# ameya-deshmukh/pbft

Measured on AMD Instinct MI355X. Metric: Ed25519 verifies/sec per node (1M-signature PBFT rounds), higher is better.
Workload: dtype u32 (GF(2^255-19) radix 2^25.5 limbs, 32x32->64 products)

## Files before the change

pbft_amd/csrc/finish.hip:

```cpp
#include <hip/hip_runtime.h>
#include <stdint.h>

#ifndef PBFT_FIN_STAMPS
#define PBFT_FIN_STAMPS 0
#endif
#if PBFT_FIN_STAMPS
#define FIN_STAMP_WAVES 4096
__device__ uint64_t g_fin_stamp[FIN_STAMP_WAVES][12];
#define FIN_STAMP(k) \
  if (lane == 0 && wave < FIN_STAMP_WAVES) g_fin_stamp[wave][k] = __builtin_amdgcn_s_memtime()
extern "C" int pbft_debug_fin_stamps(uint64_t* out, uint32_t waves) {
  if (waves > FIN_STAMP_WAVES) waves = FIN_STAMP_WAVES;
  return (int)hipMemcpyFromSymbol(out, HIP_SYMBOL(g_fin_stamp), sizeof(uint64_t) * 12 * waves, 0,
                                  hipMemcpyDeviceToHost);
}
#else
#define FIN_STAMP(k)
#endif
#include "verify_kernels.h"


template <int FM, int LV, int W>
__global__ void __launch_bounds__(BLOCK, W) finish_kernel(const uint8_t* __restrict__ R,
                                                       uint32_t rs_stride,
                                                       const uint32_t* __restrict__ xyz,
                                                       const uint8_t* __restrict__ flags, uint64_t N,
                                                       uint64_t* __restrict__ bitmap) {
  const int lane = threadIdx.x & 63;
  const uint64_t wave = ((uint64_t)blockIdx.x * BLOCK + threadIdx.x) >> 6;
  constexpr bool PRE = PBFT_FIN_PREFETCH && ((FM <= 4 && W == 1) || FM == 1);
#if FIN_USE_TAB
  __shared__ uint64_t ds_tab[LV > 0 ? DS_TAB_ENTRIES : 1];
  if constexpr (LV > 0) {
    const uint4* src = (const uint4*)g_ds_tab.e;
    uint4* dst = (uint4*)ds_tab;
#pragma unroll
    for (int k = 0; k < DS_TAB_ENTRIES / 2 / BLOCK; ++k) dst[k * BLOCK + threadIdx.x] = src[k * BLOCK + threadIdx.x];
    if (wave * FM * 64 >= N) { __syncthreads(); return; }
  }
#else
  const uint64_t* ds_tab = nullptr;
#endif
  if (wave * FM * 64 >= N) return;
  finish_wave<FM, LV, PRE, true>(wave, lane, R, rs_stride, xyz, flags, N, bitmap, ds_tab);
}


hipError_t launch_finish(int fm, int lv, int w, const uint8_t* R, uint32_t rs_stride, const uint32_t* xyz,
                         const uint8_t* flags, uint64_t N, uint64_t* bitmap, hipStream_t st) {
#define PBFT_LAUNCH_FIN(M_, LV_, W_)                                                                           \
  hipLaunchKernelGGL((finish_kernel<M_, LV_, W_>),                                                          \
                     dim3((unsigned)((((N + 64 * M_ - 1) / (64 * M_)) * 64 + BLOCK - 1) / BLOCK)), dim3(BLOCK), 0, \
                     st, R, rs_stride, xyz, flags, N, bitmap)
  if (lv == 0) {
    if (fm == 16) PBFT_LAUNCH_FIN(16, 0, FIN_WAVES_PER_EU);
    else if (fm == 8) PBFT_LAUNCH_FIN(8, 0, FIN_WAVES_PER_EU);
    else if (fm == 4) PBFT_LAUNCH_FIN(4, 0, FIN_WAVES_PER_EU);
    else if (fm == 2) PBFT_LAUNCH_FIN(2, 0, FIN_WAVES_PER_EU);
    else PBFT_LAUNCH_FIN(1, 0, FIN_WAVES_PER_EU);
  } else if (w >= 2) {
    if (fm >= 8) PBFT_LAUNCH_FIN(8, PBFT_FIN_LV, 2);
    else if (fm == 4) PBFT_LAUNCH_FIN(4, PBFT_FIN_LV, 2);
    else if (fm == 2) PBFT_LAUNCH_FIN(2, PBFT_FIN_LV, 2);
    else PBFT_LAUNCH_FIN(1, PBFT_FIN_LV, 2);
  } else {
    if (fm == 16) PBFT_LAUNCH_FIN(16, PBFT_FIN_LV, 1);
    else if (fm == 8) PBFT_LAUNCH_FIN(8, PBFT_FIN_LV, 1);
    else if (fm == 4) PBFT_LAUNCH_FIN(4, PBFT_FIN_LV, 1);
    else if (fm == 2) PBFT_LAUNCH_FIN(2, PBFT_FIN_LV, 1);
    else PBFT_LAUNCH_FIN(1, PBFT_FIN_LV, 1);
  }
#undef PBFT_LAUNCH_FIN
  return hipGetLastError();
}


// ... 42 lines not shown
```

pbft_amd/csrc/finish_core.h:

```cpp
#pragma once
#include "verify_core.h"

#ifndef FIN_STAMP
#define FIN_STAMP(k)
#endif

__device__ __forceinline__ void load_fe(fe& f, const uint32_t* __restrict__ base, uint64_t N, uint64_t i) {
#pragma unroll
  for (int t = 0; t < 10; ++t) f.v[t] = base[(size_t)t * N + i];
}

template <int M>
struct fin_unroll {
  template <class F>
  __device__ static __forceinline__ void up(F&& f) {
    fin_unroll<M - 1>::up(f);
    f(std::integral_constant<int, M - 1>());
  }
  template <class F>
  __device__ static __forceinline__ void down(F&& f) {
    f(std::integral_constant<int, M - 1>());
    fin_unroll<M - 1>::down(f);
  }
};
// ... 18 lines not shown
#endif
#ifndef PBFT_FIN_PAR
#define PBFT_FIN_PAR 0
#endif
#ifndef PBFT_FIN_DPP
#define PBFT_FIN_DPP 0
#endif
template <int K>
__device__ __forceinline__ uint32_t tree_partner(uint32_t v) {
#if PBFT_FIN_DPP
  if constexpr (K == 0) return (uint32_t)__builtin_amdgcn_mov_dpp((int)v, 0xB1, 0xF, 0xF, false);
  else if constexpr (K == 1) return (uint32_t)__builtin_amdgcn_mov_dpp((int)v, 0x4E, 0xF, 0xF, false);
  else if constexpr (K == 2) return (uint32_t)__builtin_amdgcn_mov_dpp((int)v, 0x141, 0xF, 0xF, false);
  else if constexpr (K == 3) return (uint32_t)__builtin_amdgcn_mov_dpp((int)v, 0x140, 0xF, 0xF, false);
  else if constexpr (K == 4) return (uint32_t)__builtin_amdgcn_ds_swizzle((int)v, (0x10 << 10) | 0x1F);
  else
#endif
    return (uint32_t)__shfl_xor((int)v, 1 << K);
}


template <int FM, int LV, bool PRE, bool SYNC>
__device__ __forceinline__ void finish_wave(uint64_t wave, int lane, const uint8_t* __restrict__ R, uint32_t rs_stride,
                                            const uint32_t* __restrict__ xyz, const uint8_t* __restrict__ flags,
                                            uint64_t N, uint64_t* __restrict__ bitmap, const uint64_t* ds_tab) {
  (void)ds_tab; (void)flags;
  const uint64_t base = wave * FM * 64 + lane;
  FIN_STAMP(0);
#if PBFT_FIN_STAMPS && defined(FIN_STAMP_WAVES)
  if (lane == 0 && wave < FIN_STAMP_WAVES) g_fin_stamp[wave][6] = __builtin_amdgcn_s_memrealtime();
#endif
  const uint32_t* Xb = xyz;
  const uint32_t* Yb = xyz + 10 * N;
  const uint32_t* Zb = xyz + 20 * N;
  fe pre[FM];
  fe zs[PRE ? FM : 1], xs[PRE ? FM : 1], ys[PRE ? FM : 1];
  constexpr bool PRE_R = PRE && PBFT_FIN_PREFETCH_R;
  uint32_t rs[PRE_R ? FM : 1][8];
  bool fls[PRE_R ? FM : 1];
  fin_unroll<FM>::up([&](auto mc) {
    constexpr int m = decltype(mc)::value;
    const uint64_t i = base + (uint64_t)m * 64;
    fe z;
    if (i < N) load_fe(z, Zb, N, i); else fe_one(z);
    if constexpr (PRE) {
      zs[m] = z;
      const uint64_t ii = i < N ? i : 0;
      load_fe(xs[m], Xb, N, ii);
      load_fe(ys[m], Yb, N, ii);
      if constexpr (PRE_R) {
        load32(rs[m], R + (size_t)rs_stride * ii);
        fls[m] = flags[ii];
      }
    }
    if constexpr (m == 0) pre[0] = z;
    else fe_mulT<PBFT_FIN_PAR>(pre[m], pre[m - 1], z);
  });
  FIN_STAMP(1);
  fe inv;
  fe tq[LV > 0 ? LV : 1];
  fe t = pre[FM - 1];
  static_for<LV>([&](auto kc) {
    constexpr int k = decltype(kc)::value;
#pragma unroll
    for (int u = 0; u < 10; ++u) tq[k].v[u] = tree_partner<k>(t.v[u]);
    fe_mulT<PBFT_FIN_PAR>(t, t, tq[k]);
  });
  FIN_STAMP(2);
#if PBFT_ABL_NOINV
  inv = t;
#elif PBFT_FIN_EXP
  fe_invert<true>(inv, t);
#else
  if constexpr (LV > 0) {
#if FIN_USE_TAB
// ... 10 lines not shown
    fe_invert_var(inv, t, prof);
    if (lane == 0 && wave < FIN_STAMP_WAVES) {
      g_fin_stamp[wave][8] = prof[0]; g_fin_stamp[wave][9] = prof[1]; g_fin_stamp[wave][10] = prof[2];
    }
#else
    static_assert(LV == 6, "");
    fe_invert_var(inv, t);
#endif
  } else {
    fe_invert_gcd(inv, t);
  }
#endif
  FIN_STAMP(3);
  static_for<LV>([&](auto kc) {
    constexpr int k = LV - 1 - decltype(kc)::value;
    fe_mulT<PBFT_FIN_PAR>(inv, inv, tq[k]);
  });
  FIN_STAMP(4);
  fin_unroll<FM>::down([&](auto mc) {
    constexpr int m = decltype(mc)::value;
    const uint64_t i = base + (uint64_t)m * 64;
    const bool live = i < N;
    const uint64_t ii = live ? i : 0;
    fe zi;
    if constexpr (m > 0) {
      fe_mulT<PBFT_FIN_PAR>(zi, inv, pre[m - 1]);
      fe z;
      if constexpr (PRE) z = zs[m];
      else if (live) load_fe(z, Zb, N, ii); else fe_one(z);
      fe_mulT<PBFT_FIN_PAR>(inv, inv, z);
    } else {
      zi = inv;
    }
    fe X, Y, x, y;
    if constexpr (PRE) {
      X = xs[m];
      Y = ys[m];
    } else {
      load_fe(X, Xb, N, ii);
      load_fe(Y, Yb, N, ii);
    }
    bool fl;
    uint32_t r[8];
    if constexpr (PRE_R) {
      fl = fls[m];
#pragma unroll
      for (int t = 0; t < 8; ++t) r[t] = rs[m][t];
    } else {
      fl = flags[ii];
      load32(r, R + (size_t)rs_stride * ii);
    }
    fe_mulT<PBFT_FIN_PAR>(x, X, zi);
    fe_mulT<PBFT_FIN_PAR>(y, Y, zi);
    uint32_t xw[8], yw[8], ry[8];
    fe_to_words(xw, x);
    fe_to_words(yw, y);
    canon_y(ry, r);
    bool eq = (xw[0] & 1u) == (r[7] >> 31);
#pragma unroll
    for (int t = 0; t < 8; ++t) eq = eq && yw[t] == ry[t];
    const bool ok = live && fl && eq && !y_is_small_order(yw);
    const uint64_t vote = __ballot(ok);
    if (lane == 0 && live) bitmap[(wave * FM + m)] = vote;
  });
  FIN_STAMP(5);
#if PBFT_FIN_STAMPS && defined(FIN_STAMP_WAVES)
  if (lane == 0 && wave < FIN_STAMP_WAVES) g_fin_stamp[wave][7] = __builtin_amdgcn_s_memrealtime();
#endif
}
```

pbft_amd/csrc/pbft_verify.hip:

```cpp
#include <dlfcn.h>
#include <sched.h>
#include <hip/hip_runtime.h>
#include <sys/mman.h>
#include <rccl/rccl.h>
#include <stdio.h>
#include <stdlib.h>
#include <string.h>

#include <algorithm>
#include <atomic>
#include <chrono>
#include <mutex>
#include <random>
#include <string>
#include <type_traits>
#include <vector>

#include "../../include/pbft_verify.h"
#include "../../include/pbft_wire.h"
#include "../../include/pbft_replica.h"
#include "digest_kernels.h"
#include "verify_core.h"

using namespace pbft;
// ... 340 lines not shown
    if (c->d_stage) HIP_TRY(hipFree(c->d_stage));
    c->d_stage = nullptr;
    size_t cap = bytes + (bytes >> 2) + 4096;
    if (hipMalloc(&c->d_stage, cap) != hipSuccess) { c->stage_cap = 0; return set_err(PBFT_ENOMEM, "staging alloc"); }
    c->stage_cap = cap;
  }
  if (words > c->bitmap_cap) {
    if (c->d_bitmap) HIP_TRY(hipFree(c->d_bitmap));
    if (c->h_bitmap) HIP_TRY(hipHostFree(c->h_bitmap));
    c->d_bitmap = nullptr; c->h_bitmap = nullptr; c->h_bitmap_dev = nullptr;
    size_t cap = words + 64;
    if (hipMalloc(&c->d_bitmap, cap * 8) != hipSuccess) return set_err(PBFT_ENOMEM, "bitmap alloc");
    if (hipHostMalloc(&c->h_bitmap, cap * 8, hipHostMallocMapped | hipHostMallocCoherent) != hipSuccess)
      return set_err(PBFT_ENOMEM, "pinned bitmap alloc");
    HIP_TRY(hipHostGetDevicePointer((void**)&c->h_bitmap_dev, c->h_bitmap, 0));
    c->bitmap_cap = cap;
  }
  return PBFT_OK;
}

static constexpr int MAX_STEPS = steps<PLB, PLA_SMALL>::N;
static_assert(steps<PLB, PLA_SMALL>::N >= steps<PLB, PLA_MID>::N && steps<PLB, PLA_MID>::N >= steps<PLB, PLA_BIG>::N,
              "");
static inline size_t eidx_offset(uint64_t N) { return (121 * (size_t)N + 255) & ~(size_t)255; }
static inline size_t eidx_bytes(uint64_t N) {
  const uint64_t Npad = (N + 2 * BLOCK - 1) / (2 * BLOCK) * (2 * BLOCK);
  const size_t split4 = 8 * (size_t)((MAX_STEPS + 3) / 4) * (Npad * 4 + BLOCK);
  const size_t split8 = 8 * (size_t)((MAX_STEPS + 7) / 8) * (Npad * 8 + BLOCK);
  const size_t split = split4 > split8 ? split4 : split8;
  const size_t comb = 4 * (size_t)MAX_STEPS * Npad;
  return ((comb > split ? comb : split) + 255) & ~(size_t)255;
}
static double launch_trace_ms() {
  static const double ms = [] {
    const char* e = getenv("PBFT_LAUNCH_TRACE");
    if (!e) return -1.0;
    const double v = strtod(e, nullptr);
    return v > 1 ? v / 1000.0 : 0.3;
  }();
  return ms;
}
static bool launch_trace() { return launch_trace_ms() >= 0; }
#define LT(name, ...)                                                                                              \
  do {                                                                                                             \
    const auto lt_t0 = std::chrono::steady_clock::now();                                                           \
    __VA_ARGS__;                                                                                                   \
    if (launch_trace()) {                                                                                          \
// ... 51 lines not shown
                         const uint32_t* dMI = nullptr, uint32_t n_msg = 0, const uint64_t* dWK = nullptr,
                         uint32_t mi_stride = 1, int slot = 0) {
  if (N == 0) return PBFT_OK;
  const uint64_t blocks = (N + BLOCK - 1) / BLOCK;
  if (blocks > 0x7fffffffull) return set_err(PBFT_EINVAL, "N too large for one launch");
  int rc = slot ? ensure_work2(c, N) : ensure_work(c, N, fst != nullptr);
  if (rc) return rc;
  uint8_t* const wbase = slot ? c->d_work2 : c->d_work;
  const bool timing = c->timing && slot == 0;
  int h = 0;
  if (fst) {
    h = c->half;
    c->half ^= 1;
  }
  if (slot == 0 && c->fin_pending[h]) HIP_TRY(hipStreamWaitEvent(st, c->ev_fin[h], 0));
  if (timing) LT("rec_ev0", HIP_TRY(hipEventRecord(c->ev0, st)));
  const uint64_t W = slot ? c->work2_n : c->work_n;
  uint8_t* hw = wbase + (h ? half1_offset(W) : 0);
  const bool latency_mode = N < c->split_below;
  comb_launch_args a;
  a.R = dR; a.S = dS; a.K = (const uint8_t*)dK; a.rs_stride = rs_stride; a.k_stride = k_stride;
  a.M = dM; a.msg_len = msg_len; a.msg_stride = msg_stride; a.N = N;
  a.tabB = c->d_tabB; a.tabA = c->d_tabA; a.keys = c->d_keys; a.key_ok = c->d_key_ok; a.n_keys = c->n_keys;
  a.xyz = (uint32_t*)hw;
  a.flags = hw + 120 * N;
  a.eidx = (uint32_t*)(wbase + eidx_offset(W));
  a.bitmap = dB; a.msg_idx = dMI; a.n_msg = n_msg; a.mi_stride = mi_stride; a.latency_mode = latency_mode; a.lat_split = c->lat_split; a.st = st;
  a.pair = c->comb_pair;
  a.cus = c->cus;
  a.prio = c->comb_prio;
  a.balance = c->comb_balance;
  a.wk = (PBFT_ENV_SCHED && dMI && msg_len == PBFT_ENVELOPE_LEN) ? dWK : nullptr;
  uint32_t* xyz = a.xyz;
  uint8_t* flags = a.flags;
  LT("comb", HIP_TRY(c->pa == PLA_HUGE::P  ? launch_comb_huge(a)
                     : c->pa == PLA_BIG::P ? launch_comb_big(a)
                     : c->pa == PLA_MID::P ? launch_comb_mid(a)
                                           : launch_comb_small(a)));
  HIP_TRY(hipGetLastError());
  if (fst) {
    if (timing) HIP_TRY(hipEventRecord(c->ev1, st));
    HIP_TRY(hipEventRecord(c->ev_comb, st));
    HIP_TRY(hipStreamWaitEvent(fst, c->ev_comb, 0));
    st = fst;
  }
  if (!latency_mode) {
    const bool big = N >= ((uint64_t)1 << 19);
    int fm = big ? PBFT_FIN_FM_BIG : N > PBFT_FIN_SMALL_UPTO ? PBFT_FIN_FM_MID
                                   : N > PBFT_FIN_TINY_UPTO  ? PBFT_FIN_FM_SMALL : 1;
    int lv = fm <= PBFT_FIN_TREE_MAX_FM ? PBFT_FIN_LV : 0;
    if (c->fin_m) fm = c->fin_m;
    if (c->fin_tree >= 0) lv = c->fin_tree;
    const int fw = c->fin_waves ? c->fin_waves : (big ? PBFT_FIN_W_BIG : 1);
    LT("finish", HIP_TRY(launch_finish(fm, lv, fw, dR, rs_stride, xyz, flags, N, dB, st)));
    HIP_TRY(hipGetLastError());
  }
  if (fst) {
    HIP_TRY(hipEventRecord(c->ev_fin[h], fst));
    c->fin_pending[h] = true;
    return PBFT_OK;
  }
  if (timing) LT("rec_ev1", HIP_TRY(hipEventRecord(c->ev1, st)));
  return PBFT_OK;
}

static bool check_batch_args(const void* R, const void* S, const void* K, const void* M, uint32_t msg_len,
                             uint32_t msg_stride, uint64_t N, const void* out) {
  if (N == 0) return out != nullptr || true;
  if (!R || !S || !K || !out) return false;
  if (msg_len > 0 && !M) return false;
  if (msg_stride < msg_len) return false;
  if (msg_len > (1u << 24)) return false;
  return true;
}

struct stage_layout {
  size_t offS, offK, offM, bytes;
// ... 2339 lines not shown
```

pbft_amd/csrc/verify_core.h:

```cpp
#pragma once
#include "ge25519.h"
#include "inv25519.h"
#include "sc25519.h"
#include "sha512.h"

#include <type_traits>

namespace pbft {

template <int P_, int W_, int NB_ = 0>
struct plan {
  static_assert(P_ * W_ + NB_ >= 254 && NB_ <= P_, "windows must cover 254 bits");
  static constexpr int P = P_;
  __host__ __device__ static constexpr int width(int pos) { return pos < NB_ ? W_ + 1 : W_; }
  __host__ __device__ static constexpr uint32_t entries(int pos) { return (1u << (width(pos) - 1)) + 1u; }
  __host__ __device__ static constexpr uint32_t offset(int pos) {
    return pos <= NB_ ? (uint32_t)pos * ((1u << W_) + 1u)
                      : (uint32_t)NB_ * ((1u << W_) + 1u) + (uint32_t)(pos - NB_) * ((1u << (W_ - 1)) + 1u);
  }
  __host__ __device__ static constexpr int bitoff(int pos) {
    return pos <= NB_ ? pos * (W_ + 1) : NB_ * (W_ + 1) + (pos - NB_) * W_;
  }
  static constexpr uint32_t ENTRIES = offset(P_);
  static constexpr int ENTRY_WORDS = 32;
// ... 42 lines not shown
  }
}

FE_FN uint32_t lane_mask(bool c) {
  uint32_t m = 0u - (uint32_t)c;
#if defined(__HIP_DEVICE_COMPILE__)
  asm("" : "+v"(m));
#endif
  return m;
}

#ifndef PBFT_MADD_V2
#define PBFT_MADD_V2 1
#endif
#ifndef PBFT_CHAIN_MIN_N
#define PBFT_CHAIN_MIN_N (1u << 16)
#endif
FE_FN void fe_cneg_canon(fe& out, const fe& k, uint32_t m) {
  fe nk;
  fe_neg(nk, k);
#pragma unroll
  for (int i = 0; i < 10; ++i) out.v[i] = (k.v[i] & ~m) | (nk.v[i] & m);
}
template <bool WITH_T = true, bool CHAIN = false>
FE_FN void ge_madd_ab(ge& r, const ge& p, const fe& qa, const fe& qb, const fe& k, bool neg) {
#if PBFT_MADD_V2
  fe a, b, c, t, kk;
  fe_cneg_canon(kk, k, lane_mask(neg));
  fe_sub(t, p.Y, p.X);
  if constexpr (CHAIN) {
    fe t2;
    fe_add(t2, p.Y, p.X);
    {
      fe* const ho[3] = {&a, &b, &c};
      const fe* const fo[3] = {&t, &t2, &p.T};
      const fe* const go[3] = {&qa, &qb, &kk};
      fe_mul_chain<3>(ho, fo, go);
    }
  } else {
    fe_mul(a, t, qa);
    fe_add(t, p.Y, p.X);
    fe_mul(b, t, qb);
    fe_mul(c, p.T, kk);
  }
  fe e, f, g, h;
  fe_sub(e, b, a);
  fe_sub(f, p.Z, c);
  fe_add(g, p.Z, c);
  fe_add(h, b, a);
  if constexpr (CHAIN && WITH_T) {
    fe* const ho[4] = {&r.X, &r.Y, &r.Z, &r.T};
    const fe* const fo[4] = {&f, &h, &f, &h};
    const fe* const go[4] = {&e, &g, &g, &e};
    fe_mul_chain<4>(ho, fo, go);
  } else if constexpr (CHAIN) {
    fe* const ho[3] = {&r.X, &r.Y, &r.Z};
    const fe* const fo[3] = {&f, &h, &f};
    const fe* const go[3] = {&e, &g, &g};
    fe_mul_chain<3>(ho, fo, go);
  } else {
    fe_mul(r.X, f, e);
    fe_mul(r.Y, h, g);
    fe_mul(r.Z, f, g);
    if constexpr (WITH_T) fe_mul(r.T, h, e);
  }
#else
  fe a, b, c, t;
  const uint32_t m = lane_mask(neg);
  fe_sub(t, p.Y, p.X);
  fe_mul(a, t, qa);
  fe_add(t, p.Y, p.X);
  fe_mul(b, t, qb);
// ... 89 lines not shown
#pragma unroll
  for (int i = 0; i < 8; ++i) {
    z = z && y[i] == 0u;
    one = one && y[i] == (i == 0 ? 1u : 0u);
    m1 = m1 && y[i] == (i == 0 ? 0xffffffecu : (i == 7 ? 0x7fffffffu : 0xffffffffu));
    a8 = a8 && y[i] == Y8A[i];
    b8 = b8 && y[i] == Y8B[i];
  }
  return z || one || m1 || a8 || b8;
}

FE_FN void canon_y(uint32_t y[8], const uint32_t enc[8]) {
#pragma unroll
  for (int i = 0; i < 8; ++i) y[i] = enc[i];
  y[7] &= 0x7fffffffu;
  bool ge = y[7] == 0x7fffffffu && y[0] >= 0xffffffedu;
#pragma unroll
  for (int i = 1; i < 7; ++i) ge = ge && y[i] == 0xffffffffu;
  if (ge) {
    y[0] -= 0xffffffedu;
#pragma unroll
    for (int i = 1; i < 8; ++i) y[i] = 0;
  }
}

template <int N, int I = 0, class F>
FE_FN void static_for(F&& f) {
  if constexpr (I < N) {
    f(std::integral_constant<int, I>());
    static_for<N, I + 1>(f);
  }
}

template <class PLB, class PLA, int LEN>
FE_FN bool verify_lane(const uint32_t r_enc[8], const uint32_t s[8], const uint32_t a_enc[8], bool key_ok,
                       const uint8_t* msg, int len, const uint32_t* tabB, const uint32_t* tabA) {
  const bool s_ok = sc_lt_L(s);
  uint32_t h[16], k[8];
  sha512_ram<LEN>(h, r_enc, a_enc, msg, len);
  sc_reduce512(k, h);

  ge P;
  digits ds, dk;
  uint32_t sc[8];
#pragma unroll
  for (int i = 0; i < 8; ++i) sc[i] = s[i];
// ... 112 lines not shown
```

pbft_amd/csrc/verify_kernels.h:

```cpp
#pragma once
#include <hip/hip_runtime.h>
#include <stdint.h>

#include <type_traits>

#include "verify_core.h"

using namespace pbft;


#define PBFT_ENVELOPE_LEN 85
#define BLOCK 256
#ifndef PBFT_PLAN_B
#define PBFT_PLAN_B 10, 25, 4
#endif
#ifndef PBFT_PLAN_A
#define PBFT_PLAN_A 14, 18, 2
#endif
using PLB = plan<PBFT_PLAN_B>;
using PLA_HUGE = plan<13, 19, 7>;
using PLA_BIG = plan<PBFT_PLAN_A>;
using PLA_MID = plan<16, 15, 14>;
using PLA_SMALL = plan<32, 7, 30>;
static_assert(PLA_HUGE::P < PLA_BIG::P && PLA_BIG::P < PLA_MID::P && PLA_MID::P < PLA_SMALL::P,
// ... 154 lines not shown
  }
}

#ifndef PBFT_COMB_STAMPS
#define PBFT_COMB_STAMPS 0
#endif
#if PBFT_COMB_STAMPS
#define COMB_STAMP_WAVES 16384
static __device__ uint64_t g_comb_stamp[COMB_STAMP_WAVES][8];
#define COMB_T() __builtin_amdgcn_s_memtime()
#define COMB_RT() __builtin_amdgcn_s_memrealtime()
#endif

static constexpr uint32_t COMB_PRIO_LDS = 64;
#ifndef PBFT_COMB_BALANCE
#define PBFT_COMB_BALANCE -1
#endif
template <int LEN, class PLA, bool CHAIN = false, int WPB = 4, bool BAL = false>
__global__ void __launch_bounds__(64 * WPB, PBFT_COMB_WAVES_PER_EU) comb_kernel(
    const uint8_t* __restrict__ R, const uint8_t* __restrict__ S, const uint8_t* __restrict__ key_idx,
    uint32_t rs_stride, uint32_t k_stride,
    const uint8_t* __restrict__ msg, uint32_t msg_len, uint32_t msg_stride, uint64_t N, uint64_t Npad,
    const uint32_t* __restrict__ tabB, const uint32_t* __restrict__ tabA, const uint32_t* __restrict__ keys,
    const uint8_t* __restrict__ key_ok, uint32_t n_keys, uint32_t* __restrict__ xyz, uint8_t* __restrict__ flags,
    uint32_t* __restrict__ eidx, const uint32_t* __restrict__ msg_idx, uint32_t n_msg, uint32_t mi_stride,
    const uint64_t* __restrict__ wk) {
  using ST = steps<PLB, PLA>;
  extern __shared__ __attribute__((aligned(16))) uint8_t lds[];
  const int lane = threadIdx.x & 63;
  const uint32_t wave = __builtin_amdgcn_readfirstlane(threadIdx.x >> 6);
  const uint32_t ebuf = (uint32_t)(uintptr_t)lds + wave * COMB_LDS_PER_WAVE;
  const uint64_t i = (uint64_t)blockIdx.x * (64 * WPB) + threadIdx.x;
  const bool live = i < N;
  const uint64_t ii = live ? i : 0;
  typename ST::mask_t sgn = 0;
  bool s_ok, kok;
  constexpr bool PRIO = WPB == 8;
  static_assert(!(PRIO && BAL), "the paired-priority form sets its priorities from its partner's progress");
  constexpr int BAL_J1 = ST::N / 3, BAL_J2 = 2 * ST::N / 3;
  if constexpr (BAL) __builtin_amdgcn_s_setprio(3);
  const uint32_t prog = (uint32_t)(uintptr_t)lds + WPB * COMB_LDS_PER_WAVE;
  if constexpr (PRIO) {
    if (lane == 0) lds_write32(prog + 4u * wave, 0u);
    __syncthreads();
  }
#if PBFT_COMB_STAMPS
  const uint64_t st_t0 = COMB_T(), st_rt0 = COMB_RT();
// ... 101 lines not shown
    }
    COMB_WAIT_VM();
    lds_entry_signed(rd0, neg, qa, qb, k);
    COMB_WAIT_LGKM();
    if constexpr (PRIO) {
      if ((uint32_t)j > (uint32_t)__builtin_amdgcn_readfirstlane((int)partner)) __builtin_amdgcn_s_setprio(0);
      else __builtin_amdgcn_s_setprio(2);
    }
    dma_entry_lines(ST::is_a(j + 1) ? tA : tB, nidx, lane, ebuf);
    if (j + 2 < ST::N) nidx = eidx[(size_t)(j + 2) * Npad + i];
#if PBFT_ABL_NOMADD
#pragma unroll
    for (int t = 0; t < 10; ++t) { P.X.v[t] ^= qa.v[t]; P.Y.v[t] ^= qb.v[t]; P.Z.v[t] += k.v[t] + neg; }
#else
    ge_madd_ab<true, CHAIN>(P, P, qa, qb, k, neg);
#endif
#if PBFT_LAUNDER
#pragma unroll
    for (int t = 0; t < 10; ++t) {
      asm("" : "+v"(P.X.v[t]), "+v"(P.Y.v[t]), "+v"(P.Z.v[t]), "+v"(P.T.v[t]));
    }
#endif
  }
  {
    fe qa, qb, k;
    const bool neg = (uint32_t)(sgn >> (ST::N - 1)) & 1u;
    COMB_WAIT_VM();
    lds_entry_signed(rd0, neg, qa, qb, k);
    if constexpr (PRIO) {
      if (lane == 0) lds_write32(prog + 4u * wave, 0xFFFFu);
    }
    ge_madd_ab<false, CHAIN>(P, P, qa, qb, k, neg);
  }
#if PBFT_COMB_STAMPS
  {
    const uint64_t t_end = COMB_T(), rt_end = COMB_RT();
    const uint64_t gw = (uint64_t)blockIdx.x * WPB + wave;
    if (lane == 0 && gw < COMB_STAMP_WAVES) {
      uint64_t* o = g_comb_stamp[gw];
      o[0] = st_t0; o[1] = st_rt0; o[2] = st_hash;
      o[3] = (st_wait & 0xFFFFFFFFu) | (st_first << 32);
      o[4] = t_end; o[5] = rt_end; o[6] = st_lgkm;
      o[7] = (uint64_t)__builtin_amdgcn_s_getreg((4 << 0) | (0 << 6) | (31 << 11)) |
             ((uint64_t)__builtin_amdgcn_s_getreg((20 << 0) | (0 << 6) | (31 << 11)) << 32);
    }
  }
#endif
#undef COMB_WAIT_VM
#undef COMB_WAIT_LGKM
  if (live) {
#pragma unroll
    for (int t = 0; t < 10; ++t) {
      xyz[(size_t)t * N + i] = P.X.v[t];
      xyz[(size_t)(10 + t) * N + i] = P.Y.v[t];
      xyz[(size_t)(20 + t) * N + i] = P.Z.v[t];
    }
    flags[i] = (s_ok && kok) ? 1 : 0;
  }
}

#ifndef PBFT_PAIR_MIN_N
#define PBFT_PAIR_MIN_N 0u
#endif
#ifndef PBFT_PAIR_MAX_N
#define PBFT_PAIR_MAX_N (3u << 15)
#endif
static constexpr uint32_t PAIR_SIGS = BLOCK / 2;
static constexpr uint32_t PAIR_XLDS = 8 * 64 * 4;
static constexpr size_t PAIR_LDS = (BLOCK / 64) * COMB_LDS_PER_WAVE + (BLOCK / 128) * PAIR_XLDS;
#ifndef PBFT_PAIR_A0_ADJ
#define PBFT_PAIR_A0_ADJ 0
#endif
#ifndef PBFT_PAIR_BAR
#define PBFT_PAIR_BAR 0
#endif
#ifndef PBFT_PAIR_FLIP
#define PBFT_PAIR_FLIP 0
#endif
template <class PLA>
struct pair_split {
  static constexpr int PB = PLB::P, PA = PLA::P;
  static constexpr int A0r = (PB + PA - 6) / 2 + PBFT_PAIR_A0_ADJ;
  static constexpr int BAR = PBFT_PAIR_BAR ? PBFT_PAIR_BAR : PB - 2;
  static constexpr int A0 = A0r < 1 ? 1 : A0r > PA - 1 ? PA - 1 : A0r;
  static constexpr int N1 = PB + PA - A0;
  static_assert(BAR >= 1 && BAR <= PB - 2 && N1 <= 32, "role 1 waits before its first key-position index read; "
                "its sign mask is 32 bits");
};

template <int LEN, class PLA>
__global__ void __launch_bounds__(BLOCK, PBFT_COMB_WAVES_PER_EU) comb_pair_kernel(
    const uint8_t* __restrict__ R, const uint8_t* __restrict__ S, const uint8_t* __restrict__ key_idx,
    uint32_t rs_stride, uint32_t k_stride,
    const uint8_t* __restrict__ msg, uint32_t msg_len, uint32_t msg_stride, uint64_t N, uint64_t Npad,
    const uint32_t* __restrict__ tabB, const uint32_t* __restrict__ tabA, const uint32_t* __restrict__ keys,
    const uint8_t* __restrict__ key_ok, uint32_t n_keys, uint32_t* __restrict__ xyz, uint8_t* __restrict__ flags,
    uint32_t* __restrict__ eidx, const uint32_t* __restrict__ msg_idx, uint32_t n_msg, uint32_t mi_stride,
    const uint64_t* __restrict__ wk) {
  using SP = pair_split<PLA>;
  constexpr int PB = SP::PB, PA = SP::PA, A0 = SP::A0, N1 = SP::N1;
  extern __shared__ __attribute__((aligned(16))) uint8_t lds[];
  const int lane = threadIdx.x & 63;
  const uint32_t wave = __builtin_amdgcn_readfirstlane(threadIdx.x >> 6);
  const uint32_t flip = PBFT_PAIR_FLIP ? (uint32_t)__builtin_popcount(blockIdx.x) & 1u : 0u;
  const uint32_t pair = wave >> 1, role = (wave & 1) ^ flip;
  const uint32_t lds0 = (uint32_t)(uintptr_t)lds;
  const uint32_t ebuf = lds0 + wave * COMB_LDS_PER_WAVE;
  const uint32_t pbuf = lds0 + (2 * pair + (1 ^ flip)) * COMB_LDS_PER_WAVE;
  const uint32_t xbuf = lds0 + (BLOCK / 64) * COMB_LDS_PER_WAVE + pair * PAIR_XLDS;
  const uint64_t i = (uint64_t)blockIdx.x * PAIR_SIGS + pair * 64 + lane;
  const bool live = i < N;
  const uint64_t ii = live ? i : 0;
  const uint8_t* tB = (const uint8_t*)tabB;
  const uint8_t* tA = (const uint8_t*)tabA;
  const uint32_t rd0 = ebuf + 128u * lane + 16u * (lane & 7);
  uint32_t* const erow = eidx + i;
  ge P;
  uint32_t sgn = 0;
  bool s_ok = false;
// ... 100 lines not shown
  };
  auto mul1 = [](fe& h, const fe& f, const fe& g) {
    fe* const ho[1] = {&h};
    const fe* const fo[1] = {&f};
    const fe* const go[1] = {&g};
    fe_mul_chain<1>(ho, fo, go);
  };
  fe a, b, c, t, u, w;
  lds_fe(u, 1);
  lds_fe(w, 0);
  fe_sub(t, P.Y, P.X); fe_carry(t);
  fe_sub(a, u, w); fe_carry(a);
  mul1(a, t, a);
  fe_add(t, P.Y, P.X);
  fe_add(b, u, w);
  mul1(b, t, b);
  lds_fe(u, 3);
  mul1(c, P.T, u);
  fe_const_2d(w);
  mul1(c, c, w);
  lds_fe(u, 2);
  mul1(t, P.Z, u);
  fe_add(t, t, t);
  fe e, f, g, h;
  fe_sub(e, b, a); fe_sub(f, t, c); fe_add(g, t, c); fe_add(h, b, a);
  fe_carry(e); fe_carry(f); fe_carry(g); fe_carry(h);
  fe X3, Y3, Z3;
  {
    fe* const ho[3] = {&X3, &Y3, &Z3};
    const fe* const fo[3] = {&e, &g, &f};
    const fe* const go[3] = {&f, &h, &g};
    fe_mul_chain<3>(ho, fo, go);
  }
  if (live) {
#pragma unroll
    for (int q = 0; q < 10; ++q) {
      xyz[(size_t)q * N + i] = X3.v[q];
      xyz[(size_t)(10 + q) * N + i] = Y3.v[q];
      xyz[(size_t)(20 + q) * N + i] = Z3.v[q];
    }
  }
}

#ifndef PBFT_LAT_DECOMP
#define PBFT_LAT_DECOMP 0
#endif
#ifndef PBFT_LAT_TREE
#define PBFT_LAT_TREE 1
#endif
#ifndef PBFT_LAT_WIDE_UPTO
#define PBFT_LAT_WIDE_UPTO 8192
#endif
static constexpr uint64_t LAT_WIDE_UPTO = PBFT_LAT_WIDE_UPTO;
static constexpr int LAT_COMB_WAVES = PBFT_LAT_DECOMP ? 3 : 4;
#ifndef PBFT_LAT_TAB
#define PBFT_LAT_TAB (PBFT_LAT_TREE && !PBFT_LAT_DECOMP)
#endif
#ifndef PBFT_LAT_ROWS
#define PBFT_LAT_ROWS 1
#endif
static constexpr int LAT_BLOCK = 4 * 64;
#ifndef PBFT_SPLIT_BELOW
#define PBFT_SPLIT_BELOW 12288
#endif
// ... 234 lines not shown
    acc = r == 0 && live && s_ok && kok && eq && !y_is_small_order(yw);
  }
#endif
  const uint64_t vote = __ballot(acc);
  uint32_t bits = 0;
#pragma unroll
  for (int j = 0; j < LAT_SW; ++j) bits |= (uint32_t)((vote >> (SPLIT * j)) & 1u) << j;
  const uint64_t piece = (uint64_t)blockIdx.x * LAT_COMB_WAVES + wave;
  if (lane == 0 && piece < (uint64_t)SPLIT * ((N + 63) / 64)) {
    if constexpr (LAT_SW == 16) ((uint16_t*)bitmap)[piece] = (uint16_t)bits;
    else ((uint8_t*)bitmap)[piece] = (uint8_t)bits;
  }
}

struct comb_launch_args {
  const uint8_t *R, *S, *K;
  uint32_t rs_stride, k_stride;
  const uint8_t* M;
  uint32_t msg_len, msg_stride;
  uint64_t N;
  const uint32_t *tabB, *tabA, *keys;
  const uint8_t* key_ok;
  uint32_t n_keys;
  uint32_t* xyz;
  uint8_t* flags;
  uint32_t* eidx;
  uint64_t* bitmap;
  const uint32_t* msg_idx;
  uint32_t mi_stride = 1;
  uint32_t n_msg;
  const uint64_t* wk;
  bool latency_mode;
  int lat_split;
  int pair = -1;
  int cus = 0;
  int prio = -1;
  int balance = -1;
  hipStream_t st;
};

static inline size_t comb_spread_lds(uint64_t blocks, int cus, size_t lds_min) {
  if (cus <= 0 || blocks == 0) return lds_min;
  const uint64_t per = (blocks + (uint64_t)cus - 1) / (uint64_t)cus;
  const size_t want = per == 1 ? 96 * 1024 : per == 2 ? 72 * 1024 : per == 3 ? 48 * 1024 : 0;
  return want > lds_min ? want : lds_min;
}

// ... 21 lines not shown
    const uint64_t sblocks = (pieces + LAT_COMB_WAVES - 1) / LAT_COMB_WAVES, Lpad = sblocks * LAT_COMB_WAVES * 64;
#define PBFT_LAUNCH_LAT(LEN_, SPL_)                                                                               \
  hipLaunchKernelGGL((comb_latency_kernel<LEN_, PLA, SPL_>), dim3((unsigned)sblocks), dim3(LAT_BLOCK), LAT_LDS, a.st, \
                     a.R, a.S, a.K, a.rs_stride, a.k_stride, a.M, a.msg_len, a.msg_stride, N, Lpad, a.tabB, a.tabA,   \
                     a.keys, a.key_ok, a.n_keys, a.bitmap, (const uint8_t**)a.eidx, a.msg_idx, a.n_msg, a.mi_stride, a.wk)
    if (a.msg_len == PBFT_ENVELOPE_LEN) {
      if (split == 8 && !PBFT_LAT_DECOMP) PBFT_LAUNCH_LAT(PBFT_ENVELOPE_LEN, 8 - 4 * PBFT_LAT_DECOMP);
      else PBFT_LAUNCH_LAT(PBFT_ENVELOPE_LEN, 4);
    } else {
      if (split == 8 && !PBFT_LAT_DECOMP) PBFT_LAUNCH_LAT(-1, 8 - 4 * PBFT_LAT_DECOMP);
      else PBFT_LAUNCH_LAT(-1, 4);
    }
#undef PBFT_LAUNCH_LAT
  } else {
    const uint64_t blocks = (N + BLOCK - 1) / BLOCK, Npad = blocks * BLOCK;
    const bool pair = comb_pair_sel(a);
    const size_t lds = comb_spread_lds(blocks, a.cus, (BLOCK / 64) * COMB_LDS_PER_WAVE);
    if (pair) {
      const uint64_t pblocks = (N + PAIR_SIGS - 1) / PAIR_SIGS;
      const size_t plds = comb_spread_lds(pblocks, a.cus, PAIR_LDS);
#define PBFT_LAUNCH_PAIR(LEN_)                                                                                     \
  hipLaunchKernelGGL((comb_pair_kernel<LEN_, PLA>), dim3((unsigned)pblocks), dim3(BLOCK), plds, a.st, a.R, a.S,     \
                     a.K, a.rs_stride, a.k_stride, a.M, a.msg_len, a.msg_stride, N, Npad, a.tabB, a.tabA, a.keys,    \
                     a.key_ok, a.n_keys, a.xyz, a.flags, a.eidx, a.msg_idx, a.n_msg, a.mi_stride, a.wk)
      if (a.msg_len == PBFT_ENVELOPE_LEN) PBFT_LAUNCH_PAIR(PBFT_ENVELOPE_LEN);
      else PBFT_LAUNCH_PAIR(-1);
#undef PBFT_LAUNCH_PAIR
    } else if (comb_chain_prio(a)) {
      const uint64_t b2 = (N + 2 * BLOCK - 1) / (2 * BLOCK), Npad2 = b2 * 2 * BLOCK;
      const size_t lds2 = 8 * COMB_LDS_PER_WAVE + COMB_PRIO_LDS;
      hipLaunchKernelGGL((comb_kernel<PBFT_ENVELOPE_LEN, PLA, true, 8>), dim3((unsigned)b2), dim3(2 * BLOCK), lds2,
                         a.st, a.R, a.S, a.K, a.rs_stride, a.k_stride, a.M, a.msg_len, a.msg_stride, N, Npad2, a.tabB,
                         a.tabA, a.keys, a.key_ok, a.n_keys, a.xyz, a.flags, a.eidx, a.msg_idx, a.n_msg, a.mi_stride,
                         a.wk);
    } else if (comb_chain_balance(a)) {
      hipLaunchKernelGGL((comb_kernel<PBFT_ENVELOPE_LEN, PLA, true, 4, true>), dim3((unsigned)blocks), dim3(BLOCK),
                         lds, a.st, a.R, a.S, a.K, a.rs_stride, a.k_stride, a.M, a.msg_len, a.msg_stride, N, Npad,
                         a.tabB, a.tabA, a.keys, a.key_ok, a.n_keys, a.xyz, a.flags, a.eidx, a.msg_idx, a.n_msg,
                         a.mi_stride, a.wk);
    } else if (comb_chain(a)) {
      hipLaunchKernelGGL((comb_kernel<PBFT_ENVELOPE_LEN, PLA, true, 4>), dim3((unsigned)blocks), dim3(BLOCK), lds,
                         a.st, a.R, a.S, a.K, a.rs_stride, a.k_stride, a.M, a.msg_len, a.msg_stride, N, Npad, a.tabB,
                         a.tabA, a.keys, a.key_ok, a.n_keys, a.xyz, a.flags, a.eidx, a.msg_idx, a.n_msg, a.mi_stride,
                         a.wk);
    } else if (a.msg_len == PBFT_ENVELOPE_LEN)
      hipLaunchKernelGGL((comb_kernel<PBFT_ENVELOPE_LEN, PLA>), dim3((unsigned)blocks), dim3(BLOCK), lds, a.st, a.R,
                         a.S, a.K, a.rs_stride, a.k_stride, a.M, a.msg_len, a.msg_stride, N, Npad, a.tabB, a.tabA,
                         a.keys, a.key_ok, a.n_keys, a.xyz, a.flags, a.eidx, a.msg_idx, a.n_msg, a.mi_stride, a.wk);
    else
      hipLaunchKernelGGL((comb_kernel<-1, PLA>), dim3((unsigned)blocks), dim3(BLOCK), lds, a.st, a.R, a.S, a.K,
                         a.rs_stride, a.k_stride, a.M, a.msg_len, a.msg_stride, N, Npad, a.tabB, a.tabA, a.keys,
                         a.key_ok, a.n_keys, a.xyz, a.flags, a.eidx, a.msg_idx, a.n_msg, a.mi_stride, a.wk);
  }
  return hipGetLastError();
}

hipError_t launch_comb_huge(const comb_launch_args& a);
hipError_t launch_comb_big(const comb_launch_args& a);
hipError_t launch_comb_mid(const comb_launch_args& a);
hipError_t launch_comb_small(const comb_launch_args& a);

hipError_t build_comb_tables(int pa, const uint32_t* d_enc, uint32_t n, int negate, uint32_t* d_tables,
                             uint8_t* d_key_ok, hipStream_t st, const uint32_t* d_slot = nullptr,
                             uint32_t* d_keys_out = nullptr, int* wrote = nullptr);

hipError_t launch_finish(int fm, int lv, int w, const uint8_t* R, uint32_t rs_stride, const uint32_t* xyz,
                         const uint8_t* flags, uint64_t N, uint64_t* bitmap, hipStream_t st);
void launch_sign(int len, dim3 grid, dim3 block, size_t lds, hipStream_t st, const uint32_t* seeds,
                 const uint16_t* seed_idx, const uint8_t* msg, uint32_t msg_len, uint32_t msg_stride, uint64_t N,
                 const uint32_t* tabB, uint32_t* R, uint32_t* S, uint32_t* pub, uint32_t n_seeds);
```

pbft_amd/roofline.py:

```python
import re

FIN_M = 8
FIN_TREE_LEVELS = 4
VALU_MAD_PEAK_PER_S = 31.19e12
MAD_CYCLES_PER_WAVE_INSTR = 4.53
MAD_CLOCK_HZ = 2.157e9
SIMDS = 256 * 4


def mad_peak_at(clock_hz: float) -> float:
    return SIMDS * 64 / MAD_CYCLES_PER_WAVE_INSTR * clock_hz


VALU_OP_PEAK_PER_S = 37.2e12
ENTRY_BYTES = 128
INPUT_BYTES = 32 + 32 + 2 + 85


INV_PRODUCTS = 18 * (4 * 9 + 4 * 10) + 100


def products_comb(pb: int, pa: int) -> int:
    return ((pb + pa - 1) * 7 + 1) * 100 + (81 + 44)


def products_per_verify(pb: int, pa: int) -> int:
    return (products_comb(pb, pa) + 5 * 100 + 2 * FIN_TREE_LEVELS * 100 // FIN_M
            + INV_PRODUCTS // ((1 << FIN_TREE_LEVELS) * FIN_M))


def gather_bytes_per_verify(pb: int, pa: int) -> int:
    return (pb + pa) * ENTRY_BYTES


def positions_from_build_info(info: str):
    m = re.search(r"PB=(\d+) PA=(\d+)", info)
    if not m:
        raise ValueError(f"unexpected build info: {info!r}")
    return int(m.group(1)), int(m.group(2))


PB = 10
PA = 13
PRODUCTS_PER_VERIFY = products_per_verify(PB, PA)
```

Baseline: 957.6 million.

## Store E,F,G,H from final madd and verify with cheaper projective check

The comb kernels now skip the final point conversion (the 3 field multiplies producing X,Y,Z from e,f,g,h) and write the four intermediate E,F,G,H values instead. The finish kernel batch-inverts G only. It compares x = E/G and tests H - F*y_R == 0 rather than computing both affine coordinates. Invalid-flag lanes substitute one for G before the inversion. This trades comb-side multiplies and one finish multiply for an extra 40 bytes per signature of global write and read traffic.

```diff
diff --git a/pbft_amd/csrc/finish.hip b/pbft_amd/csrc/finish.hip
--- a/pbft_amd/csrc/finish.hip
+++ b/pbft_amd/csrc/finish.hip
@@ -23,7 +23,7 @@
 template <int FM, int LV, int W>
 __global__ void __launch_bounds__(BLOCK, W) finish_kernel(const uint8_t* __restrict__ R,
                                                        uint32_t rs_stride,
-                                                       const uint32_t* __restrict__ xyz,
+                                                       const uint32_t* __restrict__ efgh,
                                                        const uint8_t* __restrict__ flags, uint64_t N,
                                                        uint64_t* __restrict__ bitmap) {
   const int lane = threadIdx.x & 63;
@@ -42,16 +42,16 @@
   const uint64_t* ds_tab = nullptr;
 #endif
   if (wave * FM * 64 >= N) return;
-  finish_wave<FM, LV, PRE, true>(wave, lane, R, rs_stride, xyz, flags, N, bitmap, ds_tab);
+  finish_wave<FM, LV, PRE, true>(wave, lane, R, rs_stride, efgh, flags, N, bitmap, ds_tab);
 }
 
 
-hipError_t launch_finish(int fm, int lv, int w, const uint8_t* R, uint32_t rs_stride, const uint32_t* xyz,
+hipError_t launch_finish(int fm, int lv, int w, const uint8_t* R, uint32_t rs_stride, const uint32_t* efgh,
                          const uint8_t* flags, uint64_t N, uint64_t* bitmap, hipStream_t st) {
 #define PBFT_LAUNCH_FIN(M_, LV_, W_)                                                                           \
   hipLaunchKernelGGL((finish_kernel<M_, LV_, W_>),                                                          \
                      dim3((unsigned)((((N + 64 * M_ - 1) / (64 * M_)) * 64 + BLOCK - 1) / BLOCK)), dim3(BLOCK), 0, \
-                     st, R, rs_stride, xyz, flags, N, bitmap)
+                     st, R, rs_stride, efgh, flags, N, bitmap)
   if (lv == 0) {
     if (fm == 16) PBFT_LAUNCH_FIN(16, 0, FIN_WAVES_PER_EU);
     else if (fm == 8) PBFT_LAUNCH_FIN(8, 0, FIN_WAVES_PER_EU);
diff --git a/pbft_amd/csrc/finish_core.h b/pbft_amd/csrc/finish_core.h
--- a/pbft_amd/csrc/finish_core.h
+++ b/pbft_amd/csrc/finish_core.h
@@ -64,35 +64,39 @@
 
 template <int FM, int LV, bool PRE, bool SYNC>
 __device__ __forceinline__ void finish_wave(uint64_t wave, int lane, const uint8_t* __restrict__ R, uint32_t rs_stride,
-                                            const uint32_t* __restrict__ xyz, const uint8_t* __restrict__ flags,
+                                            const uint32_t* __restrict__ efgh, const uint8_t* __restrict__ flags,
                                             uint64_t N, uint64_t* __restrict__ bitmap, const uint64_t* ds_tab) {
-  (void)ds_tab; (void)flags;
+  (void)ds_tab;
   const uint64_t base = wave * FM * 64 + lane;
   FIN_STAMP(0);
 #if PBFT_FIN_STAMPS && defined(FIN_STAMP_WAVES)
   if (lane == 0 && wave < FIN_STAMP_WAVES) g_fin_stamp[wave][6] = __builtin_amdgcn_s_memrealtime();
 #endif
-  const uint32_t* Xb = xyz;
-  const uint32_t* Yb = xyz + 10 * N;
-  const uint32_t* Zb = xyz + 20 * N;
+  const uint32_t* Eb = efgh;
+  const uint32_t* Fb = efgh + 10 * N;
+  const uint32_t* Gb = efgh + 20 * N;
+  const uint32_t* Hb = efgh + 30 * N;
   fe pre[FM];
-  fe zs[PRE ? FM : 1], xs[PRE ? FM : 1], ys[PRE ? FM : 1];
+  fe gs[PRE ? FM : 1], es[PRE ? FM : 1], fs[PRE ? FM : 1], hs[PRE ? FM : 1];
   constexpr bool PRE_R = PRE && PBFT_FIN_PREFETCH_R;
   uint32_t rs[PRE_R ? FM : 1][8];
-  bool fls[PRE_R ? FM : 1];
+  bool fls[PRE ? FM : 1];
   fin_unroll<FM>::up([&](auto mc) {
     constexpr int m = decltype(mc)::value;
     const uint64_t i = base + (uint64_t)m * 64;
+    const uint64_t ii = i < N ? i : 0;
+    const bool use = i < N && flags[ii];
     fe z;
-    if (i < N) load_fe(z, Zb, N, i); else fe_one(z);
+    if (i < N) load_fe(z, Gb, N, i); else fe_one(z);
+    if (!use) fe_one(z);
     if constexpr (PRE) {
-      zs[m] = z;
-      const uint64_t ii = i < N ? i : 0;
-      load_fe(xs[m], Xb, N, ii);
-      load_fe(ys[m], Yb, N, ii);
+      gs[m] = z;
+      fls[m] = use;
+      load_fe(es[m], Eb, N, ii);
+      load_fe(fs[m], Fb, N, ii);
+      load_fe(hs[m], Hb, N, ii);
       if constexpr (PRE_R) {
         load32(rs[m], R + (size_t)rs_stride * ii);
-        fls[m] = flags[ii];
       }
     }
     if constexpr (m == 0) pre[0] = z;
@@ -149,44 +153,40 @@
     const uint64_t i = base + (uint64_t)m * 64;
     const bool live = i < N;
     const uint64_t ii = live ? i : 0;
-    fe zi;
+    bool fl;
+    if constexpr (PRE) fl = fls[m];
+    else fl = live && flags[ii];
+    fe gi;
     if constexpr (m > 0) {
-      fe_mulT<PBFT_FIN_PAR>(zi, inv, pre[m - 1]);
+      fe_mulT<PBFT_FIN_PAR>(gi, inv, pre[m - 1]);
       fe z;
-      if constexpr (PRE) z = zs[m];
-      else if (live) load_fe(z, Zb, N, ii); else fe_one(z);
+      if constexpr (PRE) z = gs[m];
+      else {
+        if (live) load_fe(z, Gb, N, ii); else fe_one(z);
+        if (!fl) fe_one(z);
+      }
       fe_mulT<PBFT_FIN_PAR>(inv, inv, z);
     } else {
-      zi = inv;
+      gi = inv;
     }
-    fe X, Y, x, y;
+    fe E, F, H;
     if constexpr (PRE) {
-      X = xs[m];
-      Y = ys[m];
+      E = es[m];
+      F = fs[m];
+      H = hs[m];
     } else {
-      load_fe(X, Xb, N, ii);
-      load_fe(Y, Yb, N, ii);
+      load_fe(E, Eb, N, ii);
+      load_fe(F, Fb, N, ii);
+      load_fe(H, Hb, N, ii);
     }
-    bool fl;
     uint32_t r[8];
     if constexpr (PRE_R) {
-      fl = fls[m];
 #pragma unroll
       for (int t = 0; t < 8; ++t) r[t] = rs[m][t];
     } else {
-      fl = flags[ii];
       load32(r, R + (size_t)rs_stride * ii);
     }
-    fe_mulT<PBFT_FIN_PAR>(x, X, zi);
-    fe_mulT<PBFT_FIN_PAR>(y, Y, zi);
-    uint32_t xw[8], yw[8], ry[8];
-    fe_to_words(xw, x);
-    fe_to_words(yw, y);
-    canon_y(ry, r);
-    bool eq = (xw[0] & 1u) == (r[7] >> 31);
-#pragma unroll
-    for (int t = 0; t < 8; ++t) eq = eq && yw[t] == ry[t];
-    const bool ok = live && fl && eq && !y_is_small_order(yw);
+    const bool ok = fl && efgh_matches_r<PBFT_FIN_PAR>(E, F, H, gi, r);
     const uint64_t vote = __ballot(ok);
     if (lane == 0 && live) bitmap[(wave * FM + m)] = vote;
   });
diff --git a/pbft_amd/csrc/pbft_verify.hip b/pbft_amd/csrc/pbft_verify.hip
--- a/pbft_amd/csrc/pbft_verify.hip
+++ b/pbft_amd/csrc/pbft_verify.hip
@@ -386,7 +386,7 @@
 static constexpr int MAX_STEPS = steps<PLB, PLA_SMALL>::N;
 static_assert(steps<PLB, PLA_SMALL>::N >= steps<PLB, PLA_MID>::N && steps<PLB, PLA_MID>::N >= steps<PLB, PLA_BIG>::N,
               "");
-static inline size_t eidx_offset(uint64_t N) { return (121 * (size_t)N + 255) & ~(size_t)255; }
+static inline size_t eidx_offset(uint64_t N) { return (161 * (size_t)N + 255) & ~(size_t)255; }
 static inline size_t eidx_bytes(uint64_t N) {
   const uint64_t Npad = (N + 2 * BLOCK - 1) / (2 * BLOCK) * (2 * BLOCK);
   const size_t split4 = 8 * (size_t)((MAX_STEPS + 3) / 4) * (Npad * 4 + BLOCK);
@@ -484,8 +484,8 @@
   a.R = dR; a.S = dS; a.K = (const uint8_t*)dK; a.rs_stride = rs_stride; a.k_stride = k_stride;
   a.M = dM; a.msg_len = msg_len; a.msg_stride = msg_stride; a.N = N;
   a.tabB = c->d_tabB; a.tabA = c->d_tabA; a.keys = c->d_keys; a.key_ok = c->d_key_ok; a.n_keys = c->n_keys;
-  a.xyz = (uint32_t*)hw;
-  a.flags = hw + 120 * N;
+  a.efgh = (uint32_t*)hw;
+  a.flags = hw + 160 * N;
   a.eidx = (uint32_t*)(wbase + eidx_offset(W));
   a.bitmap = dB; a.msg_idx = dMI; a.n_msg = n_msg; a.mi_stride = mi_stride; a.latency_mode = latency_mode; a.lat_split = c->lat_split; a.st = st;
   a.pair = c->comb_pair;
@@ -493,7 +493,7 @@
   a.prio = c->comb_prio;
   a.balance = c->comb_balance;
   a.wk = (PBFT_ENV_SCHED && dMI && msg_len == PBFT_ENVELOPE_LEN) ? dWK : nullptr;
-  uint32_t* xyz = a.xyz;
+  uint32_t* efgh = a.efgh;
   uint8_t* flags = a.flags;
   LT("comb", HIP_TRY(c->pa == PLA_HUGE::P  ? launch_comb_huge(a)
                      : c->pa == PLA_BIG::P ? launch_comb_big(a)
@@ -514,7 +514,7 @@
     if (c->fin_m) fm = c->fin_m;
     if (c->fin_tree >= 0) lv = c->fin_tree;
     const int fw = c->fin_waves ? c->fin_waves : (big ? PBFT_FIN_W_BIG : 1);
-    LT("finish", HIP_TRY(launch_finish(fm, lv, fw, dR, rs_stride, xyz, flags, N, dB, st)));
+    LT("finish", HIP_TRY(launch_finish(fm, lv, fw, dR, rs_stride, efgh, flags, N, dB, st)));
     HIP_TRY(hipGetLastError());
   }
   if (fst) {
diff --git a/pbft_amd/csrc/verify_core.h b/pbft_amd/csrc/verify_core.h
--- a/pbft_amd/csrc/verify_core.h
+++ b/pbft_amd/csrc/verify_core.h
@@ -88,9 +88,9 @@
 #pragma unroll
   for (int i = 0; i < 10; ++i) out.v[i] = (k.v[i] & ~m) | (nk.v[i] & m);
 }
-template <bool WITH_T = true, bool CHAIN = false>
-FE_FN void ge_madd_ab(ge& r, const ge& p, const fe& qa, const fe& qb, const fe& k, bool neg) {
-#if PBFT_MADD_V2
+template <bool CHAIN = false>
+FE_FN void ge_madd_ab_efgh(fe& e, fe& f, fe& g, fe& h, const ge& p, const fe& qa, const fe& qb, const fe& k,
+                           bool neg) {
   fe a, b, c, t, kk;
   fe_cneg_canon(kk, k, lane_mask(neg));
   fe_sub(t, p.Y, p.X);
@@ -109,11 +109,16 @@
     fe_mul(b, t, qb);
     fe_mul(c, p.T, kk);
   }
-  fe e, f, g, h;
   fe_sub(e, b, a);
   fe_sub(f, p.Z, c);
   fe_add(g, p.Z, c);
   fe_add(h, b, a);
+}
+template <bool WITH_T = true, bool CHAIN = false>
+FE_FN void ge_madd_ab(ge& r, const ge& p, const fe& qa, const fe& qb, const fe& k, bool neg) {
+#if PBFT_MADD_V2
+  fe e, f, g, h;
+  ge_madd_ab_efgh<CHAIN>(e, f, g, h, p, qa, qb, k, neg);
   if constexpr (CHAIN && WITH_T) {
     fe* const ho[4] = {&r.X, &r.Y, &r.Z, &r.T};
     const fe* const fo[4] = {&f, &h, &f, &h};
@@ -249,6 +254,19 @@
 #pragma unroll
     for (int i = 1; i < 8; ++i) y[i] = 0;
   }
+}
+
+template <bool PAR = false>
+FE_FN bool efgh_matches_r(const fe& E, const fe& F, const fe& H, const fe& gi, const uint32_t r[8]) {
+  uint32_t ry[8], xw[8];
+  canon_y(ry, r);
+  fe x, yr, m, w;
+  fe_mulT<PAR>(x, E, gi);
+  fe_from_words(yr, ry);
+  fe_mulT<PAR>(m, F, yr);
+  fe_sub(w, H, m);
+  fe_to_words(xw, x);
+  return fe_is_zero(w) && (xw[0] & 1u) == (r[7] >> 31) && !y_is_small_order(ry);
 }
 
 template <int N, int I = 0, class F>
diff --git a/pbft_amd/csrc/verify_kernels.h b/pbft_amd/csrc/verify_kernels.h
--- a/pbft_amd/csrc/verify_kernels.h
+++ b/pbft_amd/csrc/verify_kernels.h
@@ -200,7 +200,7 @@
     uint32_t rs_stride, uint32_t k_stride,
     const uint8_t* __restrict__ msg, uint32_t msg_len, uint32_t msg_stride, uint64_t N, uint64_t Npad,
     const uint32_t* __restrict__ tabB, const uint32_t* __restrict__ tabA, const uint32_t* __restrict__ keys,
-    const uint8_t* __restrict__ key_ok, uint32_t n_keys, uint32_t* __restrict__ xyz, uint8_t* __restrict__ flags,
+    const uint8_t* __restrict__ key_ok, uint32_t n_keys, uint32_t* __restrict__ efgh, uint8_t* __restrict__ flags,
     uint32_t* __restrict__ eidx, const uint32_t* __restrict__ msg_idx, uint32_t n_msg, uint32_t mi_stride,
     const uint64_t* __restrict__ wk) {
   using ST = steps<PLB, PLA>;
@@ -348,6 +348,7 @@
     }
 #endif
   }
+  fe E, F, G, H;
   {
     fe qa, qb, k;
     const bool neg = (uint32_t)(sgn >> (ST::N - 1)) & 1u;
@@ -356,7 +357,7 @@
     if constexpr (PRIO) {
       if (lane == 0) lds_write32(prog + 4u * wave, 0xFFFFu);
     }
-    ge_madd_ab<false, CHAIN>(P, P, qa, qb, k, neg);
+    ge_madd_ab_efgh<CHAIN>(E, F, G, H, P, qa, qb, k, neg);
   }
 #if PBFT_COMB_STAMPS
   {
@@ -377,9 +378,10 @@
   if (live) {
 #pragma unroll
     for (int t = 0; t < 10; ++t) {
-      xyz[(size_t)t * N + i] = P.X.v[t];
-      xyz[(size_t)(10 + t) * N + i] = P.Y.v[t];
-      xyz[(size_t)(20 + t) * N + i] = P.Z.v[t];
+      efgh[(size_t)t * N + i] = E.v[t];
+      efgh[(size_t)(10 + t) * N + i] = F.v[t];
+      efgh[(size_t)(20 + t) * N + i] = G.v[t];
+      efgh[(size_t)(30 + t) * N + i] = H.v[t];
     }
     flags[i] = (s_ok && kok) ? 1 : 0;
   }
@@ -420,7 +422,7 @@
     uint32_t rs_stride, uint32_t k_stride,
     const uint8_t* __restrict__ msg, uint32_t msg_len, uint32_t msg_stride, uint64_t N, uint64_t Npad,
     const uint32_t* __restrict__ tabB, const uint32_t* __restrict__ tabA, const uint32_t* __restrict__ keys,
-    const uint8_t* __restrict__ key_ok, uint32_t n_keys, uint32_t* __restrict__ xyz, uint8_t* __restrict__ flags,
+    const uint8_t* __restrict__ key_ok, uint32_t n_keys, uint32_t* __restrict__ efgh, uint8_t* __restrict__ flags,
     uint32_t* __restrict__ eidx, const uint32_t* __restrict__ msg_idx, uint32_t n_msg, uint32_t mi_stride,
     const uint64_t* __restrict__ wk) {
   using SP = pair_split<PLA>;
@@ -567,24 +569,17 @@
   lds_fe(u, 2);
   mul1(t, P.Z, u);
   fe_add(t, t, t);
-  fe e, f, g, h;
-  fe_sub(e, b, a); fe_sub(f, t, c); fe_add(g, t, c); fe_add(h, b, a);
-  fe_carry(e); fe_carry(f); fe_carry(g); fe_carry(h);
-  fe X3, Y3, Z3;
-  {
-    fe* const ho[3] = {&X3, &Y3, &Z3};
-    const fe* const fo[3] = {&e, &g, &f};
-    const fe* const go[3] = {&f, &h, &g};
-    fe_mul_chain<3>(ho, fo, go);
-  }
-  if (live) {
-#pragma unroll
-    for (int q = 0; q < 10; ++q) {
-      xyz[(size_t)q * N + i] = X3.v[q];
-      xyz[(size_t)(10 + q) * N + i] = Y3.v[q];
-      xyz[(size_t)(20 + q) * N + i] = Z3.v[q];
-    }
-  }
+  auto put = [&](int c4, const fe& v) {
+    if (live) {
+#pragma unroll
+      for (int q = 0; q < 10; ++q) efgh[(size_t)(10 * c4 + q) * N + i] = v.v[q];
+    }
+  };
+  fe o;
+  fe_sub(o, b, a); put(0, o);
+  fe_add(o, b, a); put(3, o);
+  fe_sub(o, t, c); fe_carry(o); put(1, o);
+  fe_add(o, t, c); fe_carry(o); put(2, o);
 }
 
 #ifndef PBFT_LAT_DECOMP
@@ -865,7 +860,7 @@
   const uint32_t *tabB, *tabA, *keys;
   const uint8_t* key_ok;
   uint32_t n_keys;
-  uint32_t* xyz;
+  uint32_t* efgh;
   uint8_t* flags;
   uint32_t* eidx;
   uint64_t* bitmap;
@@ -933,7 +928,7 @@
 #define PBFT_LAUNCH_PAIR(LEN_)                                                                                     \
   hipLaunchKernelGGL((comb_pair_kernel<LEN_, PLA>), dim3((unsigned)pblocks), dim3(BLOCK), plds, a.st, a.R, a.S,     \
                      a.K, a.rs_stride, a.k_stride, a.M, a.msg_len, a.msg_stride, N, Npad, a.tabB, a.tabA, a.keys,    \
-                     a.key_ok, a.n_keys, a.xyz, a.flags, a.eidx, a.msg_idx, a.n_msg, a.mi_stride, a.wk)
+                     a.key_ok, a.n_keys, a.efgh, a.flags, a.eidx, a.msg_idx, a.n_msg, a.mi_stride, a.wk)
       if (a.msg_len == PBFT_ENVELOPE_LEN) PBFT_LAUNCH_PAIR(PBFT_ENVELOPE_LEN);
       else PBFT_LAUNCH_PAIR(-1);
 #undef PBFT_LAUNCH_PAIR
@@ -942,26 +937,26 @@
       const size_t lds2 = 8 * COMB_LDS_PER_WAVE + COMB_PRIO_LDS;
       hipLaunchKernelGGL((comb_kernel<PBFT_ENVELOPE_LEN, PLA, true, 8>), dim3((unsigned)b2), dim3(2 * BLOCK), lds2,
                          a.st, a.R, a.S, a.K, a.rs_stride, a.k_stride, a.M, a.msg_len, a.msg_stride, N, Npad2, a.tabB,
-                         a.tabA, a.keys, a.key_ok, a.n_keys, a.xyz, a.flags, a.eidx, a.msg_idx, a.n_msg, a.mi_stride,
+                         a.tabA, a.keys, a.key_ok, a.n_keys, a.efgh, a.flags, a.eidx, a.msg_idx, a.n_msg, a.mi_stride,
                          a.wk);
     } else if (comb_chain_balance(a)) {
       hipLaunchKernelGGL((comb_kernel<PBFT_ENVELOPE_LEN, PLA, true, 4, true>), dim3((unsigned)blocks), dim3(BLOCK),
                          lds, a.st, a.R, a.S, a.K, a.rs_stride, a.k_stride, a.M, a.msg_len, a.msg_stride, N, Npad,
-                         a.tabB, a.tabA, a.keys, a.key_ok, a.n_keys, a.xyz, a.flags, a.eidx, a.msg_idx, a.n_msg,
+                         a.tabB, a.tabA, a.keys, a.key_ok, a.n_keys, a.efgh, a.flags, a.eidx, a.msg_idx, a.n_msg,
                          a.mi_stride, a.wk);
     } else if (comb_chain(a)) {
       hipLaunchKernelGGL((comb_kernel<PBFT_ENVELOPE_LEN, PLA, true, 4>), dim3((unsigned)blocks), dim3(BLOCK), lds,
                          a.st, a.R, a.S, a.K, a.rs_stride, a.k_stride, a.M, a.msg_len, a.msg_stride, N, Npad, a.tabB,
-                         a.tabA, a.keys, a.key_ok, a.n_keys, a.xyz, a.flags, a.eidx, a.msg_idx, a.n_msg, a.mi_stride,
+                         a.tabA, a.keys, a.key_ok, a.n_keys, a.efgh, a.flags, a.eidx, a.msg_idx, a.n_msg, a.mi_stride,
                          a.wk);
     } else if (a.msg_len == PBFT_ENVELOPE_LEN)
       hipLaunchKernelGGL((comb_kernel<PBFT_ENVELOPE_LEN, PLA>), dim3((unsigned)blocks), dim3(BLOCK), lds, a.st, a.R,
                          a.S, a.K, a.rs_stride, a.k_stride, a.M, a.msg_len, a.msg_stride, N, Npad, a.tabB, a.tabA,
-                         a.keys, a.key_ok, a.n_keys, a.xyz, a.flags, a.eidx, a.msg_idx, a.n_msg, a.mi_stride, a.wk);
+                         a.keys, a.key_ok, a.n_keys, a.efgh, a.flags, a.eidx, a.msg_idx, a.n_msg, a.mi_stride, a.wk);
     else
       hipLaunchKernelGGL((comb_kernel<-1, PLA>), dim3((unsigned)blocks), dim3(BLOCK), lds, a.st, a.R, a.S, a.K,
                          a.rs_stride, a.k_stride, a.M, a.msg_len, a.msg_stride, N, Npad, a.tabB, a.tabA, a.keys,
-                         a.key_ok, a.n_keys, a.xyz, a.flags, a.eidx, a.msg_idx, a.n_msg, a.mi_stride, a.wk);
+                         a.key_ok, a.n_keys, a.efgh, a.flags, a.eidx, a.msg_idx, a.n_msg, a.mi_stride, a.wk);
   }
   return hipGetLastError();
 }
@@ -975,7 +970,7 @@
                              uint8_t* d_key_ok, hipStream_t st, const uint32_t* d_slot = nullptr,
                              uint32_t* d_keys_out = nullptr, int* wrote = nullptr);
 
-hipError_t launch_finish(int fm, int lv, int w, const uint8_t* R, uint32_t rs_stride, const uint32_t* xyz,
+hipError_t launch_finish(int fm, int lv, int w, const uint8_t* R, uint32_t rs_stride, const uint32_t* efgh,
                          const uint8_t* flags, uint64_t N, uint64_t* bitmap, hipStream_t st);
 void launch_sign(int len, dim3 grid, dim3 block, size_t lds, hipStream_t st, const uint32_t* seeds,
                  const uint16_t* seed_idx, const uint8_t* msg, uint32_t msg_len, uint32_t msg_stride, uint64_t N,
diff --git a/pbft_amd/roofline.py b/pbft_amd/roofline.py
--- a/pbft_amd/roofline.py
+++ b/pbft_amd/roofline.py
@@ -21,7 +21,7 @@
 
 
 def products_comb(pb: int, pa: int) -> int:
-    return ((pb + pa - 1) * 7 + 1) * 100 + (81 + 44)
+    return ((pb + pa - 2) * 7 + 1 + 3) * 100 + (81 + 44)
 
 
 def products_per_verify(pb: int, pa: int) -> int:
```

Result: no change. 957.5 million (-0.0%).
